# nreHieW/Eagle

Hardware: AMD Instinct MI355X
Metric: frames/sec end-to-end (detect+keypoint+homography) @1280x720 (higher is better)
Workload: dtype f32 (split: hi/lo binary16 pairs, 3 x fp16 MFMA per product, fp32 accumulate); detector (1.4 % of the FLOP): f32, exact v_mfma_f32_16x16x4_f32 chains

## Files before the change

eagle_amd/csrc/conv_ad_split32.inc:

```
#ifndef EAGLE_CONV_AD_SPLIT32_INC
#define EAGLE_CONV_AD_SPLIT32_INC
#ifndef EAGLE_ABL_M32
#define EAGLE_ABL_M32 0
#endif
#ifndef EAGLE_M32_RES_NT
#define EAGLE_M32_RES_NT 1
#endif
#ifndef EAGLE_M32_SAUX
#define EAGLE_M32_SAUX (EAGLE_STORE_NT * 2 + EAGLE_M32_RES_NT * 4)
#endif
using f32x16 = __attribute__((ext_vector_type(16))) float;
#if EAGLE_ABL_M32 == 1 || EAGLE_ABL_M32 == 6
__device__ __forceinline__ f32x16 abl_m32_xor(const half8& a_, const half8& b_, f32x16 c_)
{
    const u32x4 ua = __builtin_bit_cast(u32x4, a_), ub = __builtin_bit_cast(u32x4, b_);
    c_[0] = __builtin_bit_cast(float, __builtin_bit_cast(unsigned, c_[0]) ^ ua[0] ^ ub[3]);
    return c_;
}
#define EAGLE_MFMA_M32(A_, B_, C_) abl_m32_xor(A_, B_, C_)
#else
#define EAGLE_MFMA_M32(A_, B_, C_) __builtin_amdgcn_mfma_f32_32x32x16_f16(A_, B_, C_, 0, 0, 0)
#endif
__device__ __forceinline__ void split_store4x(char* dhi, char* dlo, float v0, float v1, float v2, float v3)
{
    const float s0 = __builtin_amdgcn_fmed3f(v0 * SPLIT_SX, -65504.0f, 65504.0f), s1 = __builtin_amdgcn_fmed3f(v1 * SPLIT_SX, -65504.0f, 65504.0f),
                s2 = __builtin_amdgcn_fmed3f(v2 * SPLIT_SX, -65504.0f, 65504.0f), s3 = __builtin_amdgcn_fmed3f(v3 * SPLIT_SX, -65504.0f, 65504.0f);
    const half4 hi = {(_Float16)s0, (_Float16)s1, (_Float16)s2, (_Float16)s3};
    const half4 lo = {(_Float16)(s0 - (float)hi[0]), (_Float16)(s1 - (float)hi[1]), (_Float16)(s2 - (float)hi[2]), (_Float16)(s3 - (float)hi[3])};
    *(half4*)dhi = hi; *(half4*)dlo = lo;
}
template <int CQ, int PG, int RES, int RING = 3, int NRH = 1>
__global__ __launch_bounds__(256, 2) void conv_split_ad32_kernel(ConvArgs a)
{
    static_assert(CQ * PG == 4, "four waves per workgroup");
    static_assert(NRH == 1 || NRH == 2, "the wave's two pixel blocks: one above the other (1) or side by side (2)");
    static_assert(18 % RING == 0 && RING >= 3, "the weight ring holds a divisor of the 18 steps of a chunk");
    using rsrc_t = __amdgpu_buffer_rsrc_t;
    constexpr unsigned OOB = 0x80000000u;
    constexpr int MB = 3, NR = 2, NRV = NR / NRH, NW = 4, BN = CQ * 96, TH = NRV * PG, TW = 32 * NRH;
    constexpr int KSTEP = (BN / 32) * 1024;
    constexpr int PS = 80, SPC = 18, AHEAD = RING - 1;
    constexpr int HW_ = TW + 2, HPIX = (TH + 2) * HW_;
    constexpr int HSLABS = ((HPIX * PS + 1023) / 1024 + NW - 1) / NW * NW, HB = HSLABS * 1024, HK = HSLABS / NW;
    constexpr int RS = 32 * 4, STRIP = 32 * RS;
    extern __shared__ __attribute__((aligned(16))) char smem[];
    char* const Hb = smem;
    char* const strip = smem + 2 * HB + (threadIdx.x >> 6) * STRIP;
    const int tid = threadIdx.x, lane = tid & 63, wave = __builtin_amdgcn_readfirstlane(tid >> 6);
    const int cq = wave % CQ, pg = wave / CQ, kh = lane >> 5, lx = lane & 31;
    const int gy = a.gy, nitems = a.tiles_x * a.tiles_y * a.N * gy, nwg = gridDim.x;
    int item0, item_end;
    {
        const int b = blockIdx.x, xcd = b & 7, k = b >> 3;
        const int wgs_here = (nwg + 7 - xcd) >> 3;
        const int qn = nitems >> 3, rn = nitems & 7;
        const int x0 = xcd < rn ? xcd * (qn + 1) : rn * (qn + 1) + (xcd - rn) * qn;
        const int xc = qn + (xcd < rn ? 1 : 0);
        item0 = x0 + (int)((long)xc * k / wgs_here);
        item_end = x0 + (int)((long)xc * (k + 1) / wgs_here);
    }
    if (item0 >= item_end) return;
    const int nloc = item_end - item0, nch = a.nchunks, GC = nloc * nch;
    const rsrc_t xrs = __builtin_amdgcn_make_buffer_rsrc((void*)a.x, 0, 0x7FFFFFFF, 0x00020000);
    const rsrc_t wrs = __builtin_amdgcn_make_buffer_rsrc((void*)a.w, 0, 0x7FFFFFFF, 0x00020000);
    const rsrc_t rrs = __builtin_amdgcn_make_buffer_rsrc((void*)a.r1, 0, 0x7FFFFFFF, 0x00020000);
    const rsrc_t rrs2 = __builtin_amdgcn_make_buffer_rsrc((void*)a.r2, 0, 0x7FFFFFFF, 0x00020000);
    const rsrc_t yrs = __builtin_amdgcn_make_buffer_rsrc((void*)a.y, 0, 0x7FFFFFFF, 0x00020000);
    constexpr bool RECOMP = HK > 6;
    const int e0 = wave * 64 + lane;
    int hpk[RECOMP ? 1 : HK];
    if constexpr (!RECOMP) {
#pragma unroll
        for (int k = 0; k < HK; ++k) {
            const int e = e0 + NW * 64 * k;
            const int pix = e / 5, slot = e - pix * 5;
            const int hy = pix / HW_, hx = pix - hy * HW_;
            hpk[k] = (pix < HPIX && slot < 4) ? (hy | (hx << 8) | (((slot & 1) * 2 + (slot >> 1)) << 16)) : -1;
        }
    }
    const int bbase = ((pg * NRV) * HW_ + lx) * PS + kh * 16;
    const unsigned wlane = (unsigned)((cq * MB * 64 + lane) * 16);

    auto decode = [&](int item, int& n, int& ty, int& tx, int& nb) {
        int t = item / gy; nb = item - t * gy;
        tx = t % a.tiles_x; t /= a.tiles_x;
        ty = t % a.tiles_y; n = t / a.tiles_y;
    };
    int h_g = 0, h_ch = 0, h_item = item0;
    int h_iy0, h_ix0, h_gb;
    auto halo_origin = [&](int item) {
        int n, ty, tx, nb; decode(item, n, ty, tx, nb);
        h_iy0 = ty * TH - 1; h_ix0 = tx * TW - 1;
        h_gb = (((n * a.H + h_iy0) * a.W + h_ix0) * a.xcs + a.xoff) * 2;
    };
    halo_origin(h_item);
    auto issue_h_slab = [&](int k) {
        char* dst = Hb + (h_g & 1) * HB;
        const unsigned so = (EAGLE_ABL_M32 == 8) ? 0u : (unsigned)(h_ch * 32) * 2u;
        int hy, hx, unit; bool live;
        if constexpr (RECOMP) {
            int e = e0 + NW * 64 * k;
            asm volatile("" : "+v"(e));
            const int pix = (int)(((unsigned)e * 52429u) >> 18), slot = e - pix * 5;
            hy = HW_ == 34 ? (int)(((unsigned)pix * 1928u) >> 16) : (int)(((unsigned)pix * 993u) >> 16); hx = pix - hy * HW_;
            unit = (slot & 1) * 2 + (slot >> 1);
            live = pix < HPIX && slot < 4;
        } else {
            hy = hpk[k] & 0xFF; hx = (hpk[k] >> 8) & 0xFF; unit = (hpk[k] >> 16) & 7; live = hpk[k] >= 0;
        }
        const int iy = h_iy0 + hy, ix = h_ix0 + hx;
        const unsigned off = !(live && (unsigned)iy < (unsigned)a.H && (unsigned)ix < (unsigned)a.W) ? OOB
                             : (unsigned)(h_gb + ((hy * a.W + hx) * a.xcs + unit * 8) * 2);
        __builtin_amdgcn_raw_ptr_buffer_load_lds(xrs, (__attribute__((address_space(3))) void*)(dst + (wave + NW * k) * 1024), 16,
                                                 ((EAGLE_ABL_M32 == 3 || EAGLE_ABL_M32 == 6 || EAGLE_ABL_M32 == 7) && h_g > 0) ? OOB : off, so, 0, 0);
    };
    auto advance_h = [&]() {
        if (h_g + 1 >= GC) return;
        ++h_g;
        if (++h_ch == nch) { h_ch = 0; ++h_item; halo_origin(h_item); }
    };
    auto issue_h = [&]() {
#pragma unroll
        for (int k = 0; k < HK; ++k) issue_h_slab(k);
        advance_h();
    };
    issue_h();
    int gc = 0;
    for (int item = item0; item < item_end; ++item) {
        int n, ty, tx, nb; decode(item, n, ty, tx, nb);
        const int oy0 = ty * TH, ox0 = tx * TW;
        f32x16 acc[MB][NR];
#pragma unroll
        for (int i = 0; i < MB; ++i)
#pragma unroll
            for (int p = 0; p < NR; ++p)
#pragma unroll
                for (int r = 0; r < 16; ++r) acc[i][p][r] = 0.f;
        u32x4 A[RING][MB];
        unsigned wsrc = (unsigned)(nb * nch * SPC) * (unsigned)KSTEP;
        const unsigned wend = wsrc + (unsigned)(nch * SPC) * (unsigned)KSTEP;
        bool abl_a_done = false;
        auto load_a = [&](int slot) {
            const unsigned so = wsrc < wend ? wsrc : wend - KSTEP;
#pragma unroll
            for (int mb = 0; mb < MB; ++mb)
                if (!((EAGLE_ABL_M32 == 2 || EAGLE_ABL_M32 == 6 || EAGLE_ABL_M32 == 7) && abl_a_done)) A[slot][mb] = __builtin_amdgcn_raw_buffer_load_b128(wrs, wlane + mb * 1024, so, 0);
            wsrc += KSTEP;
        };
#pragma unroll
        for (int s = 0; s < AHEAD; ++s) load_a(s);
        abl_a_done = true;
        for (int ch = 0; ch < nch; ++ch, ++gc) {
            if constexpr (AHEAD * MB == 6) asm volatile("s_waitcnt vmcnt(6)" ::: "memory");
            else asm volatile("s_waitcnt vmcnt(15)" ::: "memory");
            static_assert(AHEAD * MB == 6 || AHEAD * MB == 15, "vmcnt literal");
            __builtin_amdgcn_s_barrier();
            issue_h();
            const char* hb = Hb + (gc & 1) * HB + bbase;
            half8 Bh[2][NR], Bl[2][NR];
            auto read_b = [&](int slot, int tap) {
                const int ky = tap / 3, kx = tap - ky * 3;
#pragma unroll
                for (int p = 0; p < NR; ++p) {
                    Bh[slot][p] = *(const half8*)(hb + ((p / NRH + ky) * HW_ + (p % NRH) * 32 + kx) * PS);
                    Bl[slot][p] = *(const half8*)(hb + ((p / NRH + ky) * HW_ + (p % NRH) * 32 + kx) * PS + 32);
                }
            };
            read_b(0, 0);
#pragma unroll
            for (int t = 0; t < 9; ++t) {
                const int bs = (EAGLE_ABL_M32 == 4 || EAGLE_ABL_M32 == 6) ? 0 : (t & 1);
                load_a((2 * t + AHEAD) % RING);
                if (t + 1 < 9 && !(EAGLE_ABL_M32 == 4 || EAGLE_ABL_M32 == 6)) read_b((t + 1) & 1, t + 1);
#pragma unroll
                for (int p = 0; p < NR; ++p)
#pragma unroll
                    for (int mb = 0; mb < MB; ++mb) acc[mb][p] = EAGLE_MFMA_M32((half8)A[(2 * t) % RING][mb], Bh[bs][p], acc[mb][p]);
#pragma unroll
                for (int p = 0; p < NR; ++p)
#pragma unroll
                    for (int mb = 0; mb < MB; ++mb) acc[mb][p] = EAGLE_MFMA_M32((half8)A[(2 * t) % RING][mb], Bl[bs][p], acc[mb][p]);
                __builtin_amdgcn_sched_barrier(0);
                load_a((2 * t + 1 + AHEAD) % RING);
#pragma unroll
                for (int p = 0; p < NR; ++p)
#pragma unroll
                    for (int mb = 0; mb < MB; ++mb) acc[mb][p] = EAGLE_MFMA_M32((half8)A[(2 * t + 1) % RING][mb], Bh[bs][p], acc[mb][p]);
                __builtin_amdgcn_sched_barrier(0);
            }
        }
        const int co0 = nb * BN + cq * 96;
        __builtin_amdgcn_sched_barrier(0);
        const float ds = a.descale;
        int pstrip[4], ppx[4];
#pragma unroll
        for (int i = 0; i < 4; ++i) {
            const int e = i * 64 + lane, px = e >> 3, u = e & 7;
            pstrip[i] = px * RS + ((u ^ (px & 7)) * 16);
            ppx[i] = px | (u << 8);
        }
        auto piece_off = [&](int pass, int i, int cs, int off) -> unsigned {
            const int row = pass / MB, mb = pass - row * MB;
            const int oy = oy0 + pg * NRV + row / NRH, ox2 = ox0 + (row % NRH) * 32 + (ppx[i] & 0xFF), u = ppx[i] >> 8;
            return (oy < a.Ho && ox2 < a.Wo) ? (unsigned)((((n * a.Ho + oy) * a.Wo + ox2) * cs + off + (co0 + mb * 32) * 2 + u * 8) * 2) : OOB;
        };
        float vmax = 0.0f;
        constexpr int NPASS = NR * MB, PB = (RES == 2 && NRH == 2) ? 2 : (RES == 2 || (RES == 1 && NRH == 2)) ? 3 : 6;
        u32x4 rres[RES >= 1 ? PB : 1][4], rres2[RES >= 2 ? PB : 1][4];
        char* const sp = strip + lx * RS + kh * 8;
        const int sw = (lx & 7) * 16;
        auto run_hi = [&](int j) -> char* { return sp + ((j * 32) ^ sw); };
        auto run_lo = [&](int j) -> char* { return sp + ((j * 32 + 16) ^ sw); };
#pragma unroll
        for (int pb0 = 0; pb0 < NPASS; pb0 += PB) {
            if (RES >= 1) {
#pragma unroll
                for (int h2 = 0; h2 < PB; ++h2)
#pragma unroll
                    for (int i = 0; i < 4; ++i) rres[h2][i] = __builtin_amdgcn_raw_buffer_load_b128(rrs, piece_off(pb0 + h2, i, a.r1cs, a.r1off), 0, (EAGLE_M32_SAUX & 4) ? 2 : 0);
            }
            if (RES >= 2) {
#pragma unroll
                for (int h2 = 0; h2 < PB; ++h2)
#pragma unroll
                    for (int i = 0; i < 4; ++i) rres2[h2][i] = __builtin_amdgcn_raw_buffer_load_b128(rrs2, piece_off(pb0 + h2, i, a.r2cs, a.r2off), 0, (EAGLE_M32_SAUX & 4) ? 2 : 0);
            }
#pragma unroll
            for (int h2 = 0; h2 < PB; ++h2) {
                const int pass = pb0 + h2, row = pass / MB, mb = pass - row * MB;
                if (RES >= 1) {
#pragma unroll
                    for (int i = 0; i < 4; ++i) *(u32x4*)(strip + pstrip[i]) = rres[h2][i];
                }
                float v[4][4];
#pragma unroll
                for (int j = 0; j < 4; ++j) {
                    const float4 bv = *(const float4*)(a.bias + co0 + mb * 32 + j * 8 + kh * 4);
                    v[j][0] = acc[mb][row][j * 4 + 0] * ds + bv.x; v[j][1] = acc[mb][row][j * 4 + 1] * ds + bv.y;
                    v[j][2] = acc[mb][row][j * 4 + 2] * ds + bv.z; v[j][3] = acc[mb][row][j * 4 + 3] * ds + bv.w;
                    if (RES >= 1) {
                        const half4 rh = *(const half4*)run_hi(j), rl = *(const half4*)run_lo(j);
#pragma unroll
                        for (int r = 0; r < 4; ++r) v[j][r] = ((float)rh[r] + (float)rl[r]) * SPLIT_RX + v[j][r];
                    }
                }
                if (RES >= 2) {
#pragma unroll
                    for (int i = 0; i < 4; ++i) *(u32x4*)(strip + pstrip[i]) = rres2[h2][i];
#pragma unroll
                    for (int j = 0; j < 4; ++j) {
                        const half4 rh = *(const half4*)run_hi(j), rl = *(const half4*)run_lo(j);
#pragma unroll
                        for (int r = 0; r < 4; ++r) v[j][r] = v[j][r] + ((float)rh[r] + (float)rl[r]) * SPLIT_RX;
                    }
                }
#pragma unroll
                for (int j = 0; j < 4; ++j) {
                    if (a.post_act == 1) {
#pragma unroll
                        for (int r = 0; r < 4; ++r) v[j][r] = v[j][r] > 0.f ? v[j][r] : 0.f;
                    }
                    split_store4x(run_hi(j), run_lo(j), v[j][0], v[j][1], v[j][2], v[j][3]);
                    vmax = split_absmax4(vmax, v[j][0], v[j][1], v[j][2], v[j][3]);
                }
#pragma unroll
                for (int i = 0; i < 4; ++i)
                    __builtin_amdgcn_raw_buffer_store_b128(*(const u32x4*)(strip + pstrip[i]), yrs, (EAGLE_ABL_M32 >= 5 && EAGLE_ABL_M32 <= 7) ? OOB : piece_off(pass, i, a.ycs, a.yoff), 0, EAGLE_M32_SAUX & 3);
            }
        }
        split_report(a.sat, n, vmax);
    }
}

#endif
```

Before: 809.5.

## Skip MFMA and epilogue work for out-of-range output rows in split conv

Adds wave-uniform checks on whether a wave's output rows fall inside the image height. Waves with no valid rows skip all compute but still keep the barrier/halo-issue cadence. Waves where only the first row block is valid run a specialised instantiation that omits B reads, MFMAs, residual loads and stores for the second row block. This cuts wasted matrix work on bottom-edge tiles, at the cost of duplicated code (larger binary, possible register-pressure changes) and a lane index recomputed via mbcnt inside the lambda.

```diff
diff --git a/eagle_amd/csrc/conv_ad_split32.inc b/eagle_amd/csrc/conv_ad_split32.inc
--- a/eagle_amd/csrc/conv_ad_split32.inc
+++ b/eagle_amd/csrc/conv_ad_split32.inc
@@ -129,13 +129,17 @@
     for (int item = item0; item < item_end; ++item) {
         int n, ty, tx, nb; decode(item, n, ty, tx, nb);
         const int oy0 = ty * TH, ox0 = tx * TW;
-        f32x16 acc[MB][NR];
-#pragma unroll
-        for (int i = 0; i < MB; ++i)
-#pragma unroll
-            for (int p = 0; p < NR; ++p)
-#pragma unroll
-                for (int r = 0; r < 16; ++r) acc[i][p][r] = 0.f;
+        const int orow0 = oy0 + pg * NRV;
+        const bool v_any = __builtin_amdgcn_readfirstlane(orow0 < a.Ho ? 1 : 0) != 0;
+        const bool v_blk1 = NRH == 2 ? true : __builtin_amdgcn_readfirstlane(orow0 + 1 < a.Ho ? 1 : 0) != 0;
+        if (__builtin_expect(!v_any, 0)) {
+            for (int ch = 0; ch < nch; ++ch, ++gc) {
+                asm volatile("s_waitcnt vmcnt(0)" ::: "memory");
+                __builtin_amdgcn_s_barrier();
+                issue_h();
+            }
+            continue;
+        }
         u32x4 A[RING][MB];
         unsigned wsrc = (unsigned)(nb * nch * SPC) * (unsigned)KSTEP;
         const unsigned wend = wsrc + (unsigned)(nch * SPC) * (unsigned)KSTEP;
@@ -150,6 +154,16 @@
 #pragma unroll
         for (int s = 0; s < AHEAD; ++s) load_a(s);
         abl_a_done = true;
+        auto run_item = [&](auto l1_tag) {
+        constexpr bool L1 = decltype(l1_tag)::value;
+        auto mm_live = [&](int p) -> bool { return p / NRH == 0 || L1; };
+        f32x16 acc[MB][NR];
+#pragma unroll
+        for (int i = 0; i < MB; ++i)
+#pragma unroll
+            for (int p = 0; p < NR; ++p)
+#pragma unroll
+                for (int r = 0; r < 16; ++r) acc[i][p][r] = 0.f;
         for (int ch = 0; ch < nch; ++ch, ++gc) {
             if constexpr (AHEAD * MB == 6) asm volatile("s_waitcnt vmcnt(6)" ::: "memory");
             else asm volatile("s_waitcnt vmcnt(15)" ::: "memory");
@@ -162,6 +176,7 @@
                 const int ky = tap / 3, kx = tap - ky * 3;
 #pragma unroll
                 for (int p = 0; p < NR; ++p) {
+                    if (!mm_live(p)) continue;
                     Bh[slot][p] = *(const half8*)(hb + ((p / NRH + ky) * HW_ + (p % NRH) * 32 + kx) * PS);
                     Bl[slot][p] = *(const half8*)(hb + ((p / NRH + ky) * HW_ + (p % NRH) * 32 + kx) * PS + 32);
                 }
@@ -173,29 +188,38 @@
                 load_a((2 * t + AHEAD) % RING);
                 if (t + 1 < 9 && !(EAGLE_ABL_M32 == 4 || EAGLE_ABL_M32 == 6)) read_b((t + 1) & 1, t + 1);
 #pragma unroll
-                for (int p = 0; p < NR; ++p)
+                for (int p = 0; p < NR; ++p) {
+                    if (!mm_live(p)) continue;
 #pragma unroll
                     for (int mb = 0; mb < MB; ++mb) acc[mb][p] = EAGLE_MFMA_M32((half8)A[(2 * t) % RING][mb], Bh[bs][p], acc[mb][p]);
-#pragma unroll
-                for (int p = 0; p < NR; ++p)
+                }
+#pragma unroll
+                for (int p = 0; p < NR; ++p) {
+                    if (!mm_live(p)) continue;
 #pragma unroll
                     for (int mb = 0; mb < MB; ++mb) acc[mb][p] = EAGLE_MFMA_M32((half8)A[(2 * t) % RING][mb], Bl[bs][p], acc[mb][p]);
+                }
                 __builtin_amdgcn_sched_barrier(0);
                 load_a((2 * t + 1 + AHEAD) % RING);
 #pragma unroll
-                for (int p = 0; p < NR; ++p)
+                for (int p = 0; p < NR; ++p) {
+                    if (!mm_live(p)) continue;
 #pragma unroll
                     for (int mb = 0; mb < MB; ++mb) acc[mb][p] = EAGLE_MFMA_M32((half8)A[(2 * t + 1) % RING][mb], Bh[bs][p], acc[mb][p]);
+                }
                 __builtin_amdgcn_sched_barrier(0);
             }
         }
         const int co0 = nb * BN + cq * 96;
         __builtin_amdgcn_sched_barrier(0);
         const float ds = a.descale;
+        int lane_e;
+        asm volatile("v_mbcnt_lo_u32_b32 %0, -1, 0\n\tv_mbcnt_hi_u32_b32 %0, -1, %0" : "=&v"(lane_e));
+        const int lx_e = lane_e & 31, kh_e = lane_e >> 5;
         int pstrip[4], ppx[4];
 #pragma unroll
         for (int i = 0; i < 4; ++i) {
-            const int e = i * 64 + lane, px = e >> 3, u = e & 7;
+            const int e = i * 64 + lane_e, px = e >> 3, u = e & 7;
             pstrip[i] = px * RS + ((u ^ (px & 7)) * 16);
             ppx[i] = px | (u << 8);
         }
@@ -205,29 +229,34 @@
             return (oy < a.Ho && ox2 < a.Wo) ? (unsigned)((((n * a.Ho + oy) * a.Wo + ox2) * cs + off + (co0 + mb * 32) * 2 + u * 8) * 2) : OOB;
         };
         float vmax = 0.0f;
-        constexpr int NPASS = NR * MB, PB = (RES == 2 && NRH == 2) ? 2 : (RES == 2 || (RES == 1 && NRH == 2)) ? 3 : 6;
+        constexpr int NPASS = NR * MB, PB = (RES == 2 && !L1) ? 1 : (RES == 2 && NRH == 2) ? 2 : (RES == 2 || (RES == 1 && NRH == 2)) ? 3 : 6;
         u32x4 rres[RES >= 1 ? PB : 1][4], rres2[RES >= 2 ? PB : 1][4];
-        char* const sp = strip + lx * RS + kh * 8;
-        const int sw = (lx & 7) * 16;
+        char* const sp = strip + lx_e * RS + kh_e * 8;
+        const int sw = (lx_e & 7) * 16;
         auto run_hi = [&](int j) -> char* { return sp + ((j * 32) ^ sw); };
         auto run_lo = [&](int j) -> char* { return sp + ((j * 32 + 16) ^ sw); };
 #pragma unroll
         for (int pb0 = 0; pb0 < NPASS; pb0 += PB) {
             if (RES >= 1) {
 #pragma unroll
-                for (int h2 = 0; h2 < PB; ++h2)
+                for (int h2 = 0; h2 < PB; ++h2) {
+                    if (!mm_live((pb0 + h2) / MB)) continue;
 #pragma unroll
                     for (int i = 0; i < 4; ++i) rres[h2][i] = __builtin_amdgcn_raw_buffer_load_b128(rrs, piece_off(pb0 + h2, i, a.r1cs, a.r1off), 0, (EAGLE_M32_SAUX & 4) ? 2 : 0);
+                }
             }
             if (RES >= 2) {
 #pragma unroll
-                for (int h2 = 0; h2 < PB; ++h2)
+                for (int h2 = 0; h2 < PB; ++h2) {
+                    if (!mm_live((pb0 + h2) / MB)) continue;
 #pragma unroll
                     for (int i = 0; i < 4; ++i) rres2[h2][i] = __builtin_amdgcn_raw_buffer_load_b128(rrs2, piece_off(pb0 + h2, i, a.r2cs, a.r2off), 0, (EAGLE_M32_SAUX & 4) ? 2 : 0);
+                }
             }
 #pragma unroll
             for (int h2 = 0; h2 < PB; ++h2) {
                 const int pass = pb0 + h2, row = pass / MB, mb = pass - row * MB;
+                if (!mm_live(row)) continue;
                 if (RES >= 1) {
 #pragma unroll
                     for (int i = 0; i < 4; ++i) *(u32x4*)(strip + pstrip[i]) = rres[h2][i];
@@ -235,7 +264,7 @@
                 float v[4][4];
 #pragma unroll
                 for (int j = 0; j < 4; ++j) {
-                    const float4 bv = *(const float4*)(a.bias + co0 + mb * 32 + j * 8 + kh * 4);
+                    const float4 bv = *(const float4*)(a.bias + co0 + mb * 32 + j * 8 + kh_e * 4);
                     v[j][0] = acc[mb][row][j * 4 + 0] * ds + bv.x; v[j][1] = acc[mb][row][j * 4 + 1] * ds + bv.y;
                     v[j][2] = acc[mb][row][j * 4 + 2] * ds + bv.z; v[j][3] = acc[mb][row][j * 4 + 3] * ds + bv.w;
                     if (RES >= 1) {
@@ -269,6 +298,10 @@
             }
         }
         split_report(a.sat, n, vmax);
+        };
+        if constexpr (NRH == 2) run_item(std::true_type{});
+        else if (__builtin_expect(v_blk1, 1)) run_item(std::true_type{});
+        else run_item(std::false_type{});
     }
 }
 
```

Result: no change. 813.5 (median of 6 runs) (+0.5%).
